# TimoLassmann/kalign

Measured on AMD Instinct MI355X. Metric: GCUPS (DP cell updates/s) on NxL synthetic MSA, higher is better.
Workload: dtype f32

## Files before the change

kalign_amd/csrc/ka_api.cpp:

```cpp
#include "ka_ctx.h"
#include "ka_marks.h"

static thread_local std::string g_err;
int fail(const std::string& m) { g_err = m; return KA_FAIL; }
__attribute__((visibility("hidden"))) int ka_fail_message(const char* m) { return fail(m); }

extern "C" const char* ka_last_error(void) { return g_err.c_str(); }
struct ka_ctx;
int ka_ctx_device_stream(ka_ctx* c, int* device, hipStream_t* stream);
extern "C" int ka_abi_version(void) { return 29; }

extern "C" int ka_ctx_create(int device, ka_ctx** out)
{
        int n = 0;
        if (hipGetDeviceCount(&n) != hipSuccess || n <= 0) return fail("no HIP device visible (the HIP path has no CPU fallback)");
        if (device < 0 || device >= n) return fail("bad device index");
        HIPCHK(hipSetDevice(device));
        ka_ctx* c = new ka_ctx();
        c->device = device;
        {
                hipDeviceProp_t prop;
                if (hipGetDeviceProperties(&prop, device) == hipSuccess && prop.multiProcessorCount > 0) c->n_cus = prop.multiProcessorCount;
        }
        hipError_t e = hipEventCreate(&c->ev0);
// ... 159 lines not shown
        D.scratch = c->d_scratch.p; D.path_arena = c->d_path_arena.p;
        D.dbg_arena = c->d_dbg_arena.p; D.dbg_off = c->d_dbg_off.p;
        D.tasks = c->d_tasks.p; D.recs = c->d_recs.p; D.subm = c->d_subm.p;
        D.ctl = (KaCtl*)c->d_ctl.p;
        D.join = c->d_join.p;
        D.gpo0 = c->scal[0]; D.gpe0 = c->scal[1]; D.tgpe0 = c->scal[2]; D.usw = c->scal[5];
        D.numseq = c->numseq; D.flags = c->flags; D.error = c->d_error.p;
        D.nres = c->nres;
        D.trace = c->h_trace;
        D.refine_mode = 0;
        D.refine_adaptive = 0;
        D.refine_trials = 3;
        D.prof_task = -1;
        D.wdfs = (c->env.no_wdfs ? 0 : 1) | (c->env.no_ls0 ? 0 : 2) | (c->env.no_inc ? 0 : 4) | (c->env.no_ldfs ? 0 : 8);
        D.prof_task = c->env.prof_task;
        D.timing = (c->flags & KA_FLAG_TIMING) ? c->d_timing.p : nullptr;
        D.max_g = std::max(1, std::min(c->max_cluster, ka_max_g_host()));
        D.q1_mode = c->env.q1 >= 0 ? c->env.q1 : (c->nres > 5 ? 4 : 0);
        D.ho_mode = c->env.ho >= 0 ? c->env.ho : 1;
        D.per_target = c->env.per;
        D.q_order = nullptr; D.q_n = 0; D.q_slots = 0; D.qw = c->env.qw; D.lw = c->env.lw; D.reuse = c->env.reuse;
        D.overlap = c->overlap_plan ? 1 : 0;
        D.hw_mode = c->env.hw ? (1 | (c->env.hw_prio << 4)) : 0;
        D.lean4 = c->env.lean4;
        D.sub_mode = c->env.subtree;
        D.mw_mode = c->env.mw;
        D.merge_batch = c->env.merge;
        D.cons_K = c->cons_K; D.cons_maxlen = c->max_len;
        D.cons_paw = c->cons_K > 0 ? c->cons_weight / (float)c->cons_K : 0.0f;
        D.cons_maps = c->d_cons_maps.p; D.cons_map_off = c->d_cons_map_off.p;
        D.colof = c->d_colof.p; D.sip = c->d_sip.p; D.sip_off = c->d_sip_off.p;
        return D;
}

static int mark_launch(ka_ctx* c, hipStream_t s = nullptr)
{
        if (!c->env.launch_ev) return KA_OK;
        while ((int)c->launch_ev.size() < c->n_launches) { hipEvent_t e; HIPCHK(hipEventCreate(&e)); c->launch_ev.push_back(e); }
        HIPCHK(hipEventRecord(c->launch_ev[c->n_launches - 1], s ? s : c->stream));
        return KA_OK;
}

static int launch_chain(ka_ctx* c, const KaTreeDev& D, bool ov, bool join_now = true)
{
        hipStream_t cs = ov ? c->s_chain : c->stream;
        KaTreeDev Dc = D;
// ... 1165 lines not shown
```

kalign_amd/csrc/ka_device.h:

```cpp
#pragma once
#include <stdint.h>
#include "kalign_amd.h"

#define KA_F 3.402823466e+38f
#define KA_REC 64

enum { KA_SS = 0, KA_SP = 1, KA_PP = 2 };
enum { KA_FWD = 0, KA_BWD = 1 };

struct KaState { float a, ga, gb; };

struct KaTaskDesc {
        int a, b, c;
        int nsip_a, nsip_b;
        int is_root;
        float gpo, gpe, tgpe;
        float soff;
        float gap_scale;
        int parent;
        int chain_need;
        int qa, qb;
        int wait_mult;
        int refine;
};
// ... 49 lines not shown
        int* error;
        int max_g;
        int mw_mode;
        int sub_mode;
        int lean4;
        int q1_mode;
        int ho_mode;
        int hw_mode;
        int reuse;
        int overlap;
        const int2* q_order;
        int q_n, q_slots;
        int qw, lw;
        int per_target;
        int cons_K;
        int cons_maxlen;
        float cons_paw;
        const int* cons_maps;
        const long long* cons_map_off;
        int* colof;
        const int* sip;
        const long long* sip_off;
        int merge_batch;
};

#define KA_NB 6
#define KA_NB_BIG 136

struct KaPairDev {
        const uint8_t* codes;
        const int* seq_off;
        const int* seq_len;
        const int* ia;
        const int* ib;
        const float* subm;
        float gpo, gpe, tgpe;
        char* scratch;
        long long scratch_stride;
        int* paths_out;
        const long long* poff;
        float* scores;
        int* error;
        int npairs;
        int pw;
        int reuse;
};
// ... 1 lines not shown
```

kalign_amd/csrc/ka_hirschberg.h:

```cpp
#pragma once

__device__ void ka_cluster_sync(TaskShared& S)
{
        __syncthreads();
        if (S.G == 1 || S.split) return;
        if (threadIdx.x == 0) {
                __builtin_amdgcn_fence(__ATOMIC_RELEASE, "agent");
                asm volatile("s_waitcnt vmcnt(0)" ::: "memory");
                S.bar_phase += 1;
                const unsigned int target = S.bar_phase * (unsigned int)S.G;
                __hip_atomic_fetch_add(&S.ctl->bar, 1u, __ATOMIC_RELAXED, __HIP_MEMORY_SCOPE_AGENT);
                int spins = 0;
                while (__hip_atomic_load(&S.ctl->bar, __ATOMIC_RELAXED, __HIP_MEMORY_SCOPE_AGENT) < target) {
                        __builtin_amdgcn_s_sleep(4);
                        if (ka_spin_expired(S.watchdog, ++spins, 1 << 24, 6)) break;
                }
                __builtin_amdgcn_fence(__ATOMIC_ACQUIRE, "agent");
        }
        __syncthreads();
}

#define KA_CRUMB(D_trace, slot, val) do { if (D_trace) { ((volatile int*)(D_trace))[slot] = (val); __threadfence_system(); } } while (0)


template <int KIND, int NRES, int NB, bool Q1 = false, bool HO = false, bool HW = false, bool RU = false>
__device__ __forceinline__ void ka_run_items(TaskShared& S, KaCtl::Lvl* const cur, const int level, const KaSub* qc, char* lds_waves,
                                             const float* tss, long long* pslot)
{
        const int tid = threadIdx.x;
        const int lane = tid & 63;
        const int wave = tid >> 6;
        {
                        const int2* items = S.items[level & 1];
                        int* prog = S.prog[level & 1];
                        const int nitems = cur->nitems;
                        const int n16 = cur->npack[0], n4 = cur->npack[1];
                        const int njobs16 = (n16 + 3) / 4, njobs4 = (n4 + 15) / 16;
                        const int2* pack16 = S.pack[level & 1][0];
                        const int2* pack4 = S.pack[level & 1][1];
                        const int ntotal = nitems + njobs16 + njobs4;
                        const int Gw = __builtin_amdgcn_readfirstlane(S.Gw), member_w = __builtin_amdgcn_readfirstlane(S.member_w);
                        const int nslots = __builtin_amdgcn_readfirstlane(KA_NW * Gw);
                        int nreg = 1;
                        if (ntotal <= nslots) {
                                const int per_wg = (ntotal + Gw - 1) / Gw;
// ... 720 lines not shown
```

kalign_amd/csrc/ka_pass.h:

```cpp
#pragma once

#include <type_traits>

typedef float float2v __attribute__((ext_vector_type(2)));
typedef float float4v __attribute__((ext_vector_type(4)));

#define KA_STRIP_ROWS 128
#define KA_STRIP1_ROWS 64
#define KA_RING_BATCH 32
#define KA_RING_SLOTS 4
#define KA_REC_CHUNKS 7
#define KA_SLOT_BYTES (KA_REC_CHUNKS * KA_RING_BATCH * 16)
#define KA_RING_BYTES (KA_RING_SLOTS * KA_SLOT_BYTES)
#define KA_WAVE_LDS 18432
#define KA_SP_STRIDE 25
#define KA_PK_RECS 128
#define KA_SP_FILL 23
#define KA_WAVE_LDS_LEAN 6144
#define KA_T_STRIDE 24

#ifndef KA_BONUS_ASM
#define KA_BONUS_ASM 1
#endif
#ifndef KA_UNTRACKED_READS
#define KA_UNTRACKED_READS 0
#endif
#define KA_WAIT_VM0 0x0F70

typedef __attribute__((address_space(3))) void* ka_lds_ptr;
typedef const __attribute__((address_space(1))) void* ka_glb_ptr;
typedef __attribute__((address_space(1))) float ka_gfloat;
typedef const __attribute__((address_space(1))) float4v ka_gfloat4c;
typedef const __attribute__((address_space(1))) unsigned char ka_gbytec;

__device__ __forceinline__ int wave_shr1_i(int x)
{
        return __builtin_amdgcn_update_dpp(x, x, 0x138, 0xf, 0xf, false);
}

__device__ __forceinline__ float wave_shr1_old(float old, float src)
{
        return __int_as_float(__builtin_amdgcn_update_dpp(__float_as_int(old), __float_as_int(src), 0x138, 0xf, 0xf, false));
}
__device__ __forceinline__ float wave_shl1_old(float old, float src)
{
        return __int_as_float(__builtin_amdgcn_update_dpp(__float_as_int(old), __float_as_int(src), 0x130, 0xf, 0xf, false));
}
template <int E>
__device__ __forceinline__ float2v ka_mul_bcast(const float2v a, const float4v& v)
{
// ... 171 lines not shown

        const unsigned wlds_u = (unsigned)(unsigned long long)wlds;
        auto ring_issue = [&](int nb) {
                if (lane < KA_RING_BATCH && nb * KA_RING_BATCH <= ncols) {
                        const int vv = min(nb * KA_RING_BATCH + lane, ncols);
                        const float* g = p2u + ((long long)REC(vv) << 6) + 32;
                        char* dst = wlds + (nb & (KA_RING_SLOTS - 1)) * (KA_RING_BATCH * 16);
#pragma unroll
                        for (int ch = 0; ch < KA_REC_CHUNKS; ++ch)
                                if (ka_chunk_used<NRES>(ch))
                                        __builtin_amdgcn_global_load_lds((ka_glb_ptr)(g + 4 * ch), (ka_lds_ptr)(dst + ch * 2048), 16, 0, 0);
                }
        };
        if (KIND == KA_PP) {
                __builtin_amdgcn_s_waitcnt(KA_WAIT_VM0);
                ring_issue(0);
                ring_issue(1);
        }
        float oA, eA, tA, oB, eB, tB, orpA, orpB;
        float2v p1v[Q == 2 ? NRES : 1];
        constexpr int NPAIR = NRES / 2;
        float2v p1p[Q == 1 ? (NPAIR > 0 ? NPAIR : 1) : 1];
        float p1last = 0.0f;
        int res1A = 0, res1B = 0;
        if (KIND == KA_SS) {
                oA = oB = -S.gpo; eA = eB = -S.gpe; tA = tB = -S.tgpe; orpA = orpB = -S.gpo;
                res1A = S.s1[iA] * KA_T_STRIDE; res1B = S.s1[iB] * KA_T_STRIDE;
        } else {
                const float* pA = S.p1 + ((long long)recA << 6);
                const float* pB = S.p1 + ((long long)recB << 6);
                oA = pA[55] * m1; eA = pA[56] * m1; tA = pA[57] * m1;
                oB = pB[55] * m1; eB = pB[56] * m1; tB = pB[57] * m1;
                orpA = S.p1[((long long)prevA << 6) + 55] * m1;
                orpB = S.p1[((long long)prevB << 6) + 55] * m1;
                if (KIND == KA_PP) {
                        constexpr int NV = (NRES + 3) / 4;
                        if constexpr (Q == 2) {
                                float4v va[NV], vb[NV];
#pragma unroll
                                for (int i = 0; i < NV; ++i) { va[i] = ((const float4v*)pA)[i]; vb[i] = ((const float4v*)pB)[i]; }
#pragma unroll
                                for (int c = 0; c < NRES; ++c) {
                                        p1v[c].x = va[c >> 2][c & 3];
                                        p1v[c].y = actB ? vb[c >> 2][c & 3] : 0.0f;
                                }
                        } else {
                                float4v va[NV];
#pragma unroll
                                for (int i = 0; i < NV; ++i) va[i] = ((const float4v*)pA)[i];
#pragma unroll
                                for (int i = 0; i < NPAIR; ++i) { p1p[i].x = va[(2 * i) >> 2][(2 * i) & 3]; p1p[i].y = va[(2 * i + 1) >> 2][(2 * i + 1) & 3]; }
                                if (NRES & 1) p1last = va[(NRES - 1) >> 2][(NRES - 1) & 3];
                        }
                } else {
                        float* tA_ = sp_tbl + (Q * lane) * KA_SP_STRIDE;
                        float4v sa[6];
#pragma unroll
                        for (int i = 0; i < 6; ++i) sa[i] = ((const float4v*)(pA + 32))[i];
#pragma unroll
                        for (int c = 0; c < KA_SP_FILL; ++c) tA_[c] = sa[c >> 2][c & 3];
                        if constexpr (Q == 2) {
                                float* tB_ = tA_ + KA_SP_STRIDE;
                                float4v sb[6];
#pragma unroll
                                for (int i = 0; i < 6; ++i) sb[i] = ((const float4v*)(pB + 32))[i];
#pragma unroll
                                for (int c = 0; c < KA_SP_FILL; ++c) tB_[c] = sb[c >> 2][c & 3];
// ... 49 lines not shown
                             "ds_read_b128 %5, %8 offset:10240\n\t"
                             "ds_read_b128 %6, %8 offset:12288"
                             : "=&v"(dstq[0]), "=&v"(dstq[1]), "=&v"(dstq[2]), "=&v"(dstq[3]), "=&v"(dstq[4]), "=&v"(dstq[5]), "=&v"(dstq[6]),
                               "+v"(dep)
                             : "v"(a)
                             : "memory");
        };
        auto ring_wait = [&](float4v* qq) {
                if (!KA_UNTRACKED_READS) {
                        if (NRES <= 8) asm volatile("" : "+v"(qq[0]), "+v"(qq[1]), "+v"(qq[5]), "+v"(qq[6]) : : "memory");
                        else asm volatile("" : "+v"(qq[0]), "+v"(qq[1]), "+v"(qq[2]), "+v"(qq[3]), "+v"(qq[4]), "+v"(qq[5]), "+v"(qq[6]) : : "memory");
                        return;
                }
                if (NRES <= 8) {
                        asm volatile("s_waitcnt lgkmcnt(0)" : "+v"(qq[0]), "+v"(qq[1]), "+v"(qq[5]), "+v"(qq[6]) : : "memory");
                        return;
                }
                asm volatile("s_waitcnt lgkmcnt(0)"
                             : "+v"(qq[0]), "+v"(qq[1]), "+v"(qq[2]), "+v"(qq[3]), "+v"(qq[4]), "+v"(qq[5]), "+v"(qq[6])
                             :
                             : "memory");
        };

        const unsigned ho_out_u = wlds_u + KA_HO_RING;
        const unsigned ho_in_u = wlds_u - KA_WAVE_LDS + KA_HO_RING;
        const unsigned ho_my_u = (unsigned)(unsigned long long)ho_ctl_w;
        auto lds_word = [&](const unsigned addr) -> int {
                int x;
                asm volatile("ds_read_b32 %0, %1\n\ts_waitcnt lgkmcnt(0)" : "=&v"(x) : "v"(addr) : "memory");
                return __builtin_amdgcn_readfirstlane(x);
        };
        auto lds_wait_for = [&](const unsigned addr, const int need) {
                int spins = 0;
                while (lds_word(addr) < need) {
                        __builtin_amdgcn_s_sleep(1);
                        if (ka_spin_expired(wdu, ++spins, 1 << 22, 5)) break;
                }
        };

        if (KIND == KA_PP) {
                __builtin_amdgcn_s_waitcnt(KA_WAIT_VM0);
                { float2v nodep = {0.0f, 0.0f}; ring_read(q[0], min(max(-lane, 0), ncols), nodep); }
        } else {
                resn = ((ka_gbytec*)s2u)[REC(min(1 + lane, ncols)) - 1];
                if (KIND == KA_SS) { scA = tss[res1A]; if (Q == 2) scB = tss[res1B]; }
                else { scA = sp_tbl[(Q * lane) * KA_SP_STRIDE]; if (Q == 2) scB = sp_tbl[(2 * lane + 1) * KA_SP_STRIDE]; }
        }

#ifdef KA_PROF
        if (pslot && lane == 0 && pslot[2] == 0) pslot[2] = __builtin_amdgcn_s_memtime();
#endif
        auto step = [&](const int t, auto st_tag, auto full_tag, auto par_tag, auto ev_tag, auto first_tag, auto lb_tag) {
                constexpr bool LASTB = decltype(lb_tag)::value;
                constexpr bool FIRST = decltype(first_tag)::value;
                constexpr bool ST = decltype(st_tag)::value;
                constexpr bool FULL = decltype(full_tag)::value;
                constexpr int P = decltype(par_tag)::value;
                constexpr bool EV = decltype(ev_tag)::value;
                const int v = t - lane;
#ifdef KA_PROF
                const long long tq0 = __builtin_amdgcn_s_memtime();
#endif

                float copen, cext, ctext;
                if (KIND == KA_PP) {
                        ring_wait(q[P]);
#ifdef KA_PROF
                        if (EV && ST && pslot && lane == 0) pslot[256 + 0] += __builtin_amdgcn_s_memtime() - tq0;
#endif
                        copen = q[P][5].w * m2; cext = q[P][6].x * m2; ctext = q[P][6].y * m2;
                } else {
                        copen = kc_open; cext = kc_ext; ctext = kc_text;
                }
                const float scA_cur = scA, scB_cur = scB;
                if (KIND != KA_PP) {
                        if (EV && (t & 63) == 0) {
                                resb = resn;
                                resn = ((ka_gbytec*)s2u)[REC(min(t + 65 + lane, ncols)) - 1];
                        } else {
                                resb = __builtin_amdgcn_update_dpp(resb, resb, 0x134, 0xf, 0xf, false);
                        }
                        res2 = __builtin_amdgcn_update_dpp(resb, res2, 0x138, 0xf, 0xf, false);
                        if (KIND == KA_SS) { scA = tss[res1A + res2]; if (Q == 2) scB = tss[res1B + res2]; }
                        else { scA = sp_tbl[(Q * lane) * KA_SP_STRIDE + res2]; if (Q == 2) scB = sp_tbl[(2 * lane + 1) * KA_SP_STRIDE + res2]; }
                }

                if (FIRST) {
                        if (!ST && t == 0) {
                                inia = inj_a; iniga = inj_ga; inigb = inj_gb;
// ... 44 lines not shown
                }
                float upa, upga, upgb;
                const float lra = (Q == 2) ? cBa : cAa, lrga = (Q == 2) ? cBga : cAga, lrgb = (Q == 2) ? cBgb : cAgb;
                if (FIRST) {
                        upa = wave_shr1_old(bta, lra); upga = wave_shr1_old(btga, lrga); upgb = wave_shr1_old(btgb, lrgb);
                } else {
                        const float nbta = wave_rol1(bta), nbtga = wave_rol1(btga), nbtgb = wave_rol1(btgb);
                        upa = wave_shr1_old(bta, lra); upga = wave_shr1_old(btga, lrga); upgb = wave_shr1_old(btgb, lrgb);
                        bta = nbta; btga = nbtga; btgb = nbtgb;
                }

                if constexpr (Q == 2) {
                        float2v acc;
                        acc.x = kmax3(dga, dgga + copen_prev, dggb + orpA);
                        acc.y = kmax3(cAa, cAga + copen_prev, cAgb + orpB);
                        if (KIND == KA_SS) {
                                acc.x += scA_cur;
                                acc.y += scB_cur;
                                if (NB) { const int jb = (dir == KA_FWD) ? (startb + v) : (endb - v); acc.x += bonA.template at<!ST>(jb); acc.y += bonB.template at<!ST>(jb); }
                        } else if (KIND == KA_SP) {
                                acc.x += scA_cur;
                                acc.y += scB_cur;
                                if (NB) { const int jb = (dir == KA_FWD) ? (startb + v) : (endb - v); acc.x += bonA.template at<!ST>(jb); acc.y += bonB.template at<!ST>(jb); }
                        } else {
                                float2v prod;
                                prod = ka_mul_bcast<(NRES - 1) & 3>(p1v[NRES - 1], q[P][(NRES - 1) >> 2]);
        #pragma unroll
                                for (int c = NRES - 1; c >= 1; --c) {
                                        float2v nprod;
                                        switch ((c - 1) & 3) {
                                        case 0: nprod = ka_mul_bcast<0>(p1v[c - 1], q[P][(c - 1) >> 2]); break;
                                        case 1: nprod = ka_mul_bcast<1>(p1v[c - 1], q[P][(c - 1) >> 2]); break;
                                        case 2: nprod = ka_mul_bcast<2>(p1v[c - 1], q[P][(c - 1) >> 2]); break;
                                        default: nprod = ka_mul_bcast<3>(p1v[c - 1], q[P][(c - 1) >> 2]); break;
                                        }
                                        acc = acc + prod;
                                        prod = nprod;
                                }
                                acc = acc + prod;
                                if (NB) { const int jb = (dir == KA_FWD) ? (startb + v) : (endb - v); acc.x += bonA.template at<!ST>(jb); acc.y += bonB.template at<!ST>(jb); }
                                {
                                __builtin_amdgcn_sched_barrier(0);
                                const int tn = t + 1;
#ifdef KA_PROF
                                const long long tq2 = __builtin_amdgcn_s_memtime();
#endif
// ... 124 lines not shown
                                } else if (rel_agent) {
                                        __builtin_amdgcn_fence(__ATOMIC_RELEASE, "agent");
                                        asm volatile("s_waitcnt vmcnt(0)" ::: "memory");
                                        if (lane == 0) __hip_atomic_store(prog + k, vL + 1, __ATOMIC_RELAXED, __HIP_MEMORY_SCOPE_AGENT);
                                } else {
                                        __builtin_amdgcn_fence(__ATOMIC_RELEASE, "workgroup");
                                        if (lane == 0) __hip_atomic_store(prog + k, vL + 1, __ATOMIC_RELAXED, __HIP_MEMORY_SCOPE_WORKGROUP);
                                }
                                }
                        }
                }
#ifdef KA_PROF
                if (EV && ST && pslot && lane == 0) pslot[256 + 7] += __builtin_amdgcn_s_memtime() - tfl0_outer;
#endif
#ifdef KA_PROF
                const long long tri0 = __builtin_amdgcn_s_memtime();
#endif
                if (KIND == KA_PP && EV && ((t + 1) & (KA_RING_BATCH - 1)) == 0) ring_issue(((t + 1) >> 5) + 1);
#ifdef KA_PROF
                if (EV && ST && pslot && lane == 0) pslot[256 + 6] += __builtin_amdgcn_s_memtime() - tri0;
#endif
        };

        auto run = [&](int& t, const int tend, auto st_tag, auto full_tag, auto first_tag, auto lb_tag) {
                constexpr bool FIRST = decltype(first_tag)::value;
                const int e4 = ncols + lastl;
                while (t < tend) {
                        const int e1 = t | 31;
                        const int e2 = (KIND == KA_PP && FIRST) ? 0x7fffffff : ((t + CBM) & ~CBM);
                        const int e3 = t + ((lastl - t) & PBM);
                        const int e5 = (t <= e4) ? e4 : 0x7fffffff;
                        const int ev = min(min(e1, e2), min(e3, e5));
                        const int fend = min(ev, tend);
                        if ((t & 1) && t < fend) {
                                step(t, st_tag, full_tag, std::integral_constant<int, 1>(), std::false_type(), first_tag, lb_tag);
                                ++t;
                        }
                        for (; t + 1 < fend; t += 2) {
                                step(t, st_tag, full_tag, std::integral_constant<int, 0>(), std::false_type(), first_tag, lb_tag);
                                step(t + 1, st_tag, full_tag, std::integral_constant<int, 1>(), std::false_type(), first_tag, lb_tag);
                        }
                        if (t < fend) {
                                step(t, st_tag, full_tag, std::integral_constant<int, 0>(), std::false_type(), first_tag, lb_tag);
                                ++t;
                        }
                        if (t < tend && t == ev) {
                                if (t & 1) step(t, st_tag, full_tag, std::integral_constant<int, 1>(), std::true_type(), first_tag, lb_tag);
                                else step(t, st_tag, full_tag, std::integral_constant<int, 0>(), std::true_type(), first_tag, lb_tag);
                                ++t;
                        }
                }
        };
        auto run_steady = [&](int& t, const int tend, auto full_tag, auto first_tag, auto lb_tag) {
                constexpr bool FIRST = decltype(first_tag)::value;
                while (t < tend) {
                        const int e1 = t | 31;
                        const int e2 = (KIND == KA_PP && FIRST) ? 0x7fffffff : ((t + CBM) & ~CBM);
                        const int e3 = t + ((lastl - t) & PBM);
                        const int ev = min(e1, min(e2, e3));
                        const int fend = min(ev, tend);
                        if ((t & 1) && t < fend) {
                                step(t, std::true_type(), full_tag, std::integral_constant<int, 1>(), std::false_type(), first_tag, lb_tag);
                                ++t;
                        }
#ifdef KA_PROF
                        const long long tpair0 = __builtin_amdgcn_s_memtime();
                        const int t_in = t;
#endif
                        for (; t + 1 < fend; t += 2) {
                                step(t, std::true_type(), full_tag, std::integral_constant<int, 0>(), std::false_type(), first_tag, lb_tag);
                                step(t + 1, std::true_type(), full_tag, std::integral_constant<int, 1>(), std::false_type(), first_tag, lb_tag);
                        }
#ifdef KA_PROF
                        if (pslot && lane == 0) { pslot[6] += __builtin_amdgcn_s_memtime() - tpair0; pslot[7] += t - t_in; }
#endif
                        if (t < fend) {
                                step(t, std::true_type(), full_tag, std::integral_constant<int, 0>(), std::false_type(), first_tag, lb_tag);
                                ++t;
                        }
#ifdef KA_PROF
                        const long long tev0 = __builtin_amdgcn_s_memtime();
                        const int ev_in = t;
#endif
                        if (t < tend && t == ev) {
                                if (t & 1) step(t, std::true_type(), full_tag, std::integral_constant<int, 1>(), std::true_type(), first_tag, lb_tag);
                                else step(t, std::true_type(), full_tag, std::integral_constant<int, 0>(), std::true_type(), first_tag, lb_tag);
                                ++t;
                        }
#ifdef KA_PROF
                        if (pslot && lane == 0) { pslot[256 + 2] += __builtin_amdgcn_s_memtime() - tev0; pslot[256 + 3] += t - ev_in; }
#endif
                }
        };

        const int nsteps = ncols + nl;
        const int t_steady0 = min(nl, nsteps);
        const int t_steady1 = ncols;
        auto phases = [&](auto full_tag, auto first_tag, auto lb_tag) {
                int t = 0;
                run(t, t_steady0, std::false_type(), full_tag, first_tag, lb_tag);
                run_steady(t, t_steady1, full_tag, first_tag, lb_tag);
                run(t, nsteps, std::false_type(), full_tag, first_tag, lb_tag);
        };
        auto go = [&](auto full_tag, auto first_tag) {
                constexpr bool FULL = decltype(full_tag)::value;
                if constexpr (FULL || Q == 1) phases(full_tag, first_tag, std::integral_constant<bool, Q == 2>());
                else { if (last_is_b) phases(full_tag, first_tag, std::true_type()); else phases(full_tag, first_tag, std::false_type()); }
        };
        if (nr == SROWS) {
                if (first) go(std::true_type(), std::true_type());
                else go(std::true_type(), std::false_type());
        } else {
                if (first) go(std::false_type(), std::true_type());
                else go(std::false_type(), std::false_type());
        }
#undef REC
#undef IDX
}

template <int KIND, int NRES, int SLOT, int NB>
__device__ __forceinline__ void ka_packed(const TaskShared& S, const KaSub* qc, const int2* pack, const int nslots,
                                          const int job, const int lane, const float* tss, char* wlds,
                                          const int nreg = 1, const int reg_stride = 0)
{
        constexpr int SPW = 64 / SLOT;
        const int slot = job * SPW + lane / SLOT;
        const int ls = lane % SLOT;
        const bool live = slot < nslots;
        const int2 d = pack[live ? slot : 0];
        const KaSub* sp = qc + d.x;
        const int dir = d.y;
        const int starta = sp->starta, enda = sp->enda, startb = sp->startb, endb = sp->endb;
        const int ncols = endb - startb;
        const int mid = ((enda - starta) / 2) + starta;
        const int r0 = (dir == KA_FWD) ? starta : mid;
        const int r1 = (dir == KA_FWD) ? mid : enda;
        const int nrows = r1 - r0;
// ... 202 lines not shown
```

kalign_amd/csrc/ka_plan.h:

```cpp
#pragma once
#define KA_INTERNAL __attribute__((visibility("hidden")))

#include <algorithm>
#include <cstdlib>
#include <string>
#include <vector>

#include "ka_device.h"

KA_INTERNAL int fail(const std::string& m);

struct KaEnv {
        bool trace = false, no_chain = false, no_queue = false, no_half = false, no_lean = false, chain_g1 = false, no_crit = false;
        bool no_staging = false, no_wdfs = false, no_ls0 = false, no_inc = false, no_ldfs = false, refine_serial = false;
        int chain_tasks = 0;
        int max_cluster = 0;
        int crit_greedy = 1;
        int crit_top = 0;
        int prof_task = -1;
        int q1 = -1;
        int lean4 = 1;
        int mw = 1;
        int merge = 15;
        int per = 0;
        int ho = -1;
        int hw = 1;
        int hw_prio = 3;
        int subtree = 1;
        int overlap = 1;
        int overlap_help = 1;
        int reuse = 1;
        int qw = 4, lw = 4, pw = 2;
        bool launch_ev = false;
        bool upgma_launches = false;
        bool qorder = true;
        bool plan_verbose = false;
};
static inline int env_int(const char* name, int dflt) { const char* e = getenv(name); return e ? atoi(e) : dflt; }
static inline void read_env(KaEnv& v)
{
        v = KaEnv();
        v.trace = getenv("KA_TRACE") != nullptr; v.no_chain = getenv("KA_NO_CHAIN") != nullptr; v.no_queue = getenv("KA_NO_QUEUE") != nullptr;
        v.no_half = getenv("KA_NO_HALF") != nullptr; v.no_lean = getenv("KA_NO_LEAN") != nullptr; v.chain_g1 = getenv("KA_CHAIN_G1") != nullptr;
        v.no_crit = getenv("KA_NO_CRIT") != nullptr; v.no_staging = getenv("KA_NO_STAGING") != nullptr;
        v.no_wdfs = getenv("KA_NO_WDFS") != nullptr; v.no_ls0 = getenv("KA_NO_LS0") != nullptr; v.no_inc = getenv("KA_NO_INC") != nullptr; v.no_ldfs = getenv("KA_NO_LDFS") != nullptr; v.refine_serial = getenv("KA_REFINE_SERIAL") != nullptr;
        v.chain_tasks = env_int("KA_CHAIN_TASKS", 0); v.max_cluster = env_int("KA_MAX_CLUSTER", 0); v.crit_top = env_int("KA_CRIT_TOP", 0); v.crit_greedy = env_int("KA_CRIT_GREEDY", 1);
        v.prof_task = env_int("KA_PROF_TASK", -1); v.q1 = env_int("KA_Q1", -1); v.lean4 = env_int("KA_LEAN4", 1);
        v.launch_ev = getenv("KA_LAUNCH_EV") != nullptr;
        v.subtree = env_int("KA_SUBTREE", 1);
        v.reuse = env_int("KA_REUSE", 1);
        v.overlap_help = env_int("KA_OVERLAP_HELP", 1);
        v.overlap = env_int("KA_OVERLAP", 1);
        v.qw = env_int("KA_QW", 4); v.lw = env_int("KA_LW", 4); v.pw = env_int("KA_PW", 2);
        for (int* w : { &v.qw, &v.lw, &v.pw }) if (*w != 1 && *w != 2) *w = 4;
        v.mw = env_int("KA_MW", 1);
        v.merge = env_int("KA_MERGE", 15);
        v.ho = env_int("KA_HO", -1);
        v.per = env_int("KA_PER", 0);
        v.hw = env_int("KA_HW", 1);
        v.hw_prio = std::max(0, std::min(3, env_int("KA_HW_PRIO", 3)));
        v.upgma_launches = getenv("KA_UPGMA_LAUNCHES") != nullptr;
        v.qorder = env_int("KA_QORDER", 1) != 0;
        v.plan_verbose = getenv("KA_PLAN_VERBOSE") != nullptr;
}

struct KaPlan {
        KaEnv env;
        int numseq = 0, n_tasks = 0;
        std::vector<int> lens;
        std::vector<int> abc;
        std::vector<KaTaskDesc> descs;
        std::vector<std::vector<int>> levels;
        std::vector<int> task_level;
        std::vector<int> sip_flat;
        std::vector<long long> sip_off;
        std::vector<char> plan_active;
        int n_cus = 256;
        bool shared_gpu = false;
        int cons_K = 0;
        int test_hooks = 0;
        std::vector<std::vector<int>> plan_levels;
        std::vector<int2> blocks_flat;
// ... 16 lines not shown
```

kalign_amd/csrc/ka_shared.h:

```cpp
#pragma once

#define KA_BLOCK 512
#define KA_WAVES (KA_BLOCK / 64)
#define KA_PAIR_BLOCK 256
#define KA_LEAN_BLOCK 512
#define KA_NT ((int)blockDim.x)
#define KA_NW ((int)blockDim.x >> 6)

__device__ __forceinline__ float kmax(float a, float b) { return fmaxf(a, b); }
__device__ __forceinline__ float kmax3(float a, float b, float c) { return fmaxf(fmaxf(a, b), c); }

__device__ __forceinline__ float wave_shr1(float x)
{
        int xi = __float_as_int(x);
        return __int_as_float(__builtin_amdgcn_update_dpp(xi, xi, 0x138, 0xf, 0xf, false));
}

__device__ __forceinline__ float ka_uniform_f(float x)
{
        return __int_as_float(__builtin_amdgcn_readfirstlane(__float_as_int(x)));
}

template <typename T>
__device__ __forceinline__ T* ka_uniform_ptr(T* p)
// ... 11 lines not shown
        return false;
}

__device__ __forceinline__ float lane_bcast(float x, int src_lane)
{
        return __int_as_float(__builtin_amdgcn_readlane(__float_as_int(x), src_lane));
}

struct KaCtl {
        struct Lvl { int nsub, rowalloc, nitems, next_item, npack[2], next_job, pad; } lvl[2];
        int mcount;
        int top_meet, top_tr;
        float top_score;
        double msum;
        int alnlen;
        int fail;
        unsigned int bar;
        int nrec;
        long long scratch_off;
        long long newp_off;
        long long path_off;
        int regalloc_pad[2];
};

struct TaskShared {
        int kind, swapped;
        int len_a, len_b;
        int La, Lb;
        const uint8_t* s1;
        const uint8_t* s2;
        const float* p1;
        const float* p2;
        float* profa;
        float* profb;
        const float* subm;
        float gpo, gpe, tgpe, soff;
        float sp_open, sp_ext, sp_text;
        float p1_mult, p2_mult;
        KaState* fbuf;
        KaState* bbuf;
        KaState* xfbuf;
        KaState* xbbuf;
        KaState* sfbuf[2];
        KaState* sbbuf[2];
        int reuse_ok;
        KaSub* q[2];
// ... 32 lines not shown
        float* mlog;
        int mlog_cap, adapt_trials;
        int2* mrec;
        char* inc;
        int inc_n, inc_nunc;
        int inc_j, inc_p;
        int rec_on;
        float sp_value;
        int Gw, member_w;
        int split;
        struct Priv { KaSub* q[2]; int2* items[2]; int* prog[2]; int2* pack[2][2]; KaState* f; KaState* b; } priv;
        unsigned int bar_phase;
        int2* items[2];
        int* prog[2];
        int2* pack[2][2];
        float* newp;
        int* path_dst;
        int* trace;
        int dbgskip;
        int* watchdog;
        long long t_pass, t_meet;
        int n_levels;
        int next_member, next_g;
        long long* prof;
        int lvl_n[16];
        int lvl_pass[16], lvl_meet[16];
};

template <int KIND>
__device__ __forceinline__ void col_terms(const TaskShared& S, int rec, float& copen, float& cext, float& ctext)
{
        if (KIND == KA_SS) { copen = -S.gpo; cext = -S.gpe; ctext = -S.tgpe; }
        else if (KIND == KA_SP) { copen = -S.sp_open; cext = -S.sp_ext; ctext = -S.sp_text; }
        else {
                const float* c = S.p2 + ((long long)rec << 6);
                copen = c[55] * S.p2_mult; cext = c[56] * S.p2_mult; ctext = c[57] * S.p2_mult;
        }
}
```

kalign_amd/csrc/ka_task.h:

```cpp
#pragma once

#ifndef KA_RU_TREE
#define KA_RU_TREE 0
#endif
#define KA_LDS_DBG 1400
#define KA_LDS_TSS 1408
#define KA_LDS_WAVES 4096
static_assert(KA_LDS_TSS + 23 * KA_T_STRIDE * 4 <= KA_LDS_WAVES - KA_LDS_HO_BACK, "score table overlaps the hand-over control words");
static_assert(KA_LDS_TSS + 23 * KA_T_STRIDE * 4 <= KA_LDS_WAVES, "score table overlaps the wave regions");
#define KA_LDS_TOTAL (KA_LDS_WAVES + KA_WAVES * KA_WAVE_LDS)
#define KA_HALF_BLOCK 256
#define KA_LDS_HALF (KA_LDS_WAVES + (KA_HALF_BLOCK / 64) * KA_WAVE_LDS)
#define KA_LEAN_SCRATCH(nt_) ((((2 * (nt_) + 16) * 4) + 15) & ~15)
#define KA_LDS_PAIR (KA_LDS_WAVES + KA_LEAN_SCRATCH(KA_PAIR_BLOCK) + (KA_PAIR_BLOCK / 64) * KA_WAVE_LDS_LEAN)
#define KA_LDS_LEAN (KA_LDS_WAVES + KA_LEAN_SCRATCH(KA_LEAN_BLOCK) + (KA_LEAN_BLOCK / 64) * KA_WAVE_LDS_LEAN)
static_assert(sizeof(TaskShared) <= KA_LDS_DBG, "TaskShared outgrew its LDS slot");
static_assert(KA_LDS_WAVES % 16 == 0, "wave regions must be 16-B aligned");

__device__ void ka_build_tss(float* tss, const float* subm, float soff)
{
        for (int x = threadIdx.x; x < 23 * KA_T_STRIDE; x += KA_NT) {
                const int a = x / KA_T_STRIDE, b = x % KA_T_STRIDE;
                tss[x] = (b < 23) ? (subm[23 * a + b] - soff) : 0.0f;
        }
// ... 194 lines not shown
                S.kind = kind; S.swapped = swapped;
                S.p1_mult = swapped ? (float)T.nsip_a : (float)T.nsip_b;
                S.p2_mult = swapped ? (float)T.nsip_b : (float)T.nsip_a;
                S.La = swapped ? len_b : len_a;
                S.Lb = swapped ? len_a : len_b;
                int g_eff = (S.La >= 1536) ? 8 : ((S.La >= 1152) ? 6 : ((S.La >= 768) ? 4 : ((S.La >= 320) ? 2 : 1)));
                int srows = KA_STRIP_ROWS;
                int q1_lvl = 0;
                if (Q1 && D.q1_mode == 4) {
                        if (D.hw_mode && kind == KA_PP) {
                                const int s1 = ka_strips_of(S.La / 2, KA_STRIP1_ROWS) + ka_strips_of(S.La - S.La / 2, KA_STRIP1_ROWS);
                                q1_lvl = 1;
                                g_eff = max(g_eff, min(g_launch, (s1 + 3) / 4));
                        }
                } else if (Q1 && D.q1_mode) {
                        const int s1 = ka_strips_of(S.La / 2, KA_STRIP1_ROWS) + ka_strips_of(S.La - S.La / 2, KA_STRIP1_ROWS);
                        const int g1 = (s1 + 3) / 4;
                        if (g1 <= g_launch || (D.q1_mode >= 2 && (s1 + 7) / 8 <= g_launch) || D.q1_mode >= 3) { srows = KA_STRIP1_ROWS; g_eff = g1; }
                }
                S.q1_lvl = q1_lvl;
                S.lvl_srows[0] = srows; S.lvl_srows[1] = srows;
                S.ho_ok = (Q1 && NB == 0 && D.ho_mode && kind == KA_PP) ? 1 : 0;
                S.hw_ok = (Q1 && D.hw_mode && kind == KA_PP) ? D.hw_mode : 0;
                if (Q1 && kind == KA_PP) {
                        const int s2 = ka_strips_of(S.La / 2, srows) + ka_strips_of(S.La - S.La / 2, srows);
                        g_eff = (S.ho_ok && D.ho_mode >= 2) ? max((s2 + 3) / 4, 1) : max(g_eff, (s2 + 3) / 4);
                        if (S.hw_ok && !q1_lvl) {
                                int need = s2;
                                for (int l = 1; l < 5; ++l) {
                                        const int rows = (S.La + (2 << l) - 1) >> (l + 1);
                                        if (rows < 2 * srows) break;
                                        need = max(need, (2 << l) * ka_strips_of(rows, srows));
                                }
                                g_eff = max(g_eff, min(g_launch, (need + 3) / 4));
                        }
                }
                if (Q1 && D.per_target > 0 && kind == KA_PP) {
                        const int s2 = ka_strips_of(S.La / 2, srows) + ka_strips_of(S.La - S.La / 2, srows);
                        g_eff = max((s2 + D.per_target - 1) / D.per_target, 1);
                }
                if (NB && D.cons_K > 0 && T.nsip_a + T.nsip_b >= 128) {
                        const int mem = max(T.nsip_a, T.nsip_b);
                        g_eff = max(g_eff, 2 * D.cons_K * (mem >= 1536 ? 3 : (mem >= 384 ? 2 : 1)));
                }
                if (g_eff > g_launch) g_eff = g_launch;
                S.srows = srows;
// ... 515 lines not shown
```

Baseline: 56.03.

## Add gathered sparse profile scoring path for low-residue-count PP rows

Adds a specialised profile-profile DP step that, when every lane's row profile has at most four nonzero residue columns, gathers only those columns from the LDS ring and computes the match score with a few multiply-adds instead of the dense NRES-wide dot product. The choice is made per strip through a wave-wide ballot, and the whole pass loop is instantiated twice via a template tag. This targets per-cell ALU and LDS read cost on near-identical synthetic MSAs, at the cost of larger code, extra register pressure, and a path that only runs in the KA_UNIT==2 build.

```diff
diff --git a/kalign_amd/csrc/ka_api.cpp b/kalign_amd/csrc/ka_api.cpp
--- a/kalign_amd/csrc/ka_api.cpp
+++ b/kalign_amd/csrc/ka_api.cpp
@@ -205,6 +205,7 @@
         D.q_order = nullptr; D.q_n = 0; D.q_slots = 0; D.qw = c->env.qw; D.lw = c->env.lw; D.reuse = c->env.reuse;
         D.overlap = c->overlap_plan ? 1 : 0;
         D.hw_mode = c->env.hw ? (1 | (c->env.hw_prio << 4)) : 0;
+        D.sparse_mode = c->env.sparse ? 1 : 0;
         D.lean4 = c->env.lean4;
         D.sub_mode = c->env.subtree;
         D.mw_mode = c->env.mw;
diff --git a/kalign_amd/csrc/ka_device.h b/kalign_amd/csrc/ka_device.h
--- a/kalign_amd/csrc/ka_device.h
+++ b/kalign_amd/csrc/ka_device.h
@@ -95,6 +95,7 @@
         const int* sip;
         const long long* sip_off;
         int merge_batch;
+        int sparse_mode;
 };
 
 #define KA_NB 6
diff --git a/kalign_amd/csrc/ka_hirschberg.h b/kalign_amd/csrc/ka_hirschberg.h
--- a/kalign_amd/csrc/ka_hirschberg.h
+++ b/kalign_amd/csrc/ka_hirschberg.h
@@ -20,7 +20,6 @@
         __syncthreads();
 }
 
-#define KA_CRUMB(D_trace, slot, val) do { if (D_trace) { ((volatile int*)(D_trace))[slot] = (val); __threadfence_system(); } } while (0)
 
 
 template <int KIND, int NRES, int NB, bool Q1 = false, bool HO = false, bool HW = false, bool RU = false>
diff --git a/kalign_amd/csrc/ka_pass.h b/kalign_amd/csrc/ka_pass.h
--- a/kalign_amd/csrc/ka_pass.h
+++ b/kalign_amd/csrc/ka_pass.h
@@ -26,6 +26,15 @@
 #define KA_UNTRACKED_READS 0
 #endif
 #define KA_WAIT_VM0 0x0F70
+
+#ifndef KA_SPARSE_NT
+#define KA_SPARSE_NT 4
+#endif
+#if defined(KA_UNIT) && KA_UNIT == 2
+#define KA_SPARSE_BUILT 1
+#else
+#define KA_SPARSE_BUILT 0
+#endif
 
 typedef __attribute__((address_space(3))) void* ka_lds_ptr;
 typedef const __attribute__((address_space(1))) void* ka_glb_ptr;
@@ -243,6 +252,12 @@
         constexpr int NPAIR = NRES / 2;
         float2v p1p[Q == 1 ? (NPAIR > 0 ? NPAIR : 1) : 1];
         float p1last = 0.0f;
+        constexpr bool SPB = KA_SPARSE_BUILT && KIND == KA_PP && NRES >= 20 && NB == 0 && Q == 2;
+        constexpr int SP_NTMAX = SPB ? KA_SPARSE_NT : 1;
+        static_assert(!SPB || !KA_UNTRACKED_READS, "the gathered form reads the ring with tracked loads only");
+        int sp_nt = 0;
+        float2v spc[SP_NTMAX];
+        unsigned spo[SP_NTMAX];
         int res1A = 0, res1B = 0;
         if (KIND == KA_SS) {
                 oA = oB = -S.gpo; eA = eB = -S.gpe; tA = tB = -S.tgpe; orpA = orpB = -S.gpo;
@@ -260,10 +275,33 @@
                                 float4v va[NV], vb[NV];
 #pragma unroll
                                 for (int i = 0; i < NV; ++i) { va[i] = ((const float4v*)pA)[i]; vb[i] = ((const float4v*)pB)[i]; }
-#pragma unroll
-                                for (int c = 0; c < NRES; ++c) {
-                                        p1v[c].x = va[c >> 2][c & 3];
-                                        p1v[c].y = actB ? vb[c >> 2][c & 3] : 0.0f;
+                                if constexpr (SPB) {
+                                        unsigned nz = 0;
+#pragma unroll
+                                        for (int c = 0; c < NRES; ++c)
+                                                if (va[c >> 2][c & 3] != 0.0f || (actB && vb[c >> 2][c & 3] != 0.0f)) nz |= 1u << c;
+                                        const int nterms = __popc(nz);
+                                        if (__builtin_amdgcn_readfirstlane(S.sparse_ok) != 0 && __ballot(nterms > KA_SPARSE_NT) == 0ull) sp_nt = KA_SPARSE_NT;
+                                        if (S.trace && lane == 0) ((volatile int*)S.trace)[sp_nt ? KA_TRACE_GATHERED : KA_TRACE_DENSE] = 1;
+                                        if (sp_nt) {
+#pragma unroll
+                                                for (int i = 0; i < SP_NTMAX; ++i) {
+                                                        const bool has = nz != 0u;
+                                                        const int c = has ? 31 - __clz(nz) : 0;
+                                                        nz &= ~(1u << c);
+                                                        const float xa = pA[c], xb = pB[c];
+                                                        spc[i].x = has ? xa : 0.0f;
+                                                        spc[i].y = (has && actB) ? xb : 0.0f;
+                                                        spo[i] = wlds_u + (unsigned)((c >> 2) * 2048 + (c & 3) * 4);
+                                                }
+                                        }
+                                }
+                                if (!SPB || sp_nt == 0) {
+#pragma unroll
+                                        for (int c = 0; c < NRES; ++c) {
+                                                p1v[c].x = va[c >> 2][c & 3];
+                                                p1v[c].y = actB ? vb[c >> 2][c & 3] : 0.0f;
+                                        }
                                 }
                         } else {
                                 float4v va[NV];
@@ -359,6 +397,25 @@
                              : "memory");
         };
 
+        float sq[2][SP_NTMAX];
+        auto sp_read = [&](float4v* dstq, float* dsts, int vcol, auto& dep, auto n_tag) {
+                constexpr int N = decltype(n_tag)::value;
+                typedef const __attribute__((address_space(3))) float4v ka_l4;
+                typedef const __attribute__((address_space(3))) float ka_l1;
+                const unsigned cb = ((unsigned)vcol & 127u) << 4;
+                ka_l4* const cr = (ka_l4*)(unsigned long)(wlds_u | cb);
+                asm volatile("" : "+v"(dep) : : "memory");
+#pragma unroll
+                for (int i = 0; i < N; ++i) dsts[i] = *(ka_l1*)(unsigned long)(spo[i] | cb);
+                dstq[5] = cr[5 * 128]; dstq[6] = cr[6 * 128];
+        };
+        auto sp_wait = [&](float4v* qq, float* ss, auto n_tag) {
+                constexpr int N = decltype(n_tag)::value;
+#pragma unroll
+                for (int i = 0; i < N; ++i) asm volatile("" : "+v"(ss[i]) : : "memory");
+                asm volatile("" : "+v"(qq[5]), "+v"(qq[6]) : : "memory");
+        };
+
         const unsigned ho_out_u = wlds_u + KA_HO_RING;
         const unsigned ho_in_u = wlds_u - KA_WAVE_LDS + KA_HO_RING;
         const unsigned ho_my_u = (unsigned)(unsigned long long)ho_ctl_w;
@@ -377,7 +434,11 @@
 
         if (KIND == KA_PP) {
                 __builtin_amdgcn_s_waitcnt(KA_WAIT_VM0);
-                { float2v nodep = {0.0f, 0.0f}; ring_read(q[0], min(max(-lane, 0), ncols), nodep); }
+                float2v nodep = {0.0f, 0.0f};
+                bool gathered = false;
+                if constexpr (SPB) gathered = sp_nt != 0;
+                if (gathered) sp_read(q[0], sq[0], min(max(-lane, 0), ncols), nodep, std::integral_constant<int, SP_NTMAX>());
+                else ring_read(q[0], min(max(-lane, 0), ncols), nodep);
         } else {
                 resn = ((ka_gbytec*)s2u)[REC(min(1 + lane, ncols)) - 1];
                 if (KIND == KA_SS) { scA = tss[res1A]; if (Q == 2) scB = tss[res1B]; }
@@ -387,7 +448,8 @@
 #ifdef KA_PROF
         if (pslot && lane == 0 && pslot[2] == 0) pslot[2] = __builtin_amdgcn_s_memtime();
 #endif
-        auto step = [&](const int t, auto st_tag, auto full_tag, auto par_tag, auto ev_tag, auto first_tag, auto lb_tag) {
+        auto step = [&](const int t, auto st_tag, auto full_tag, auto par_tag, auto ev_tag, auto first_tag, auto lb_tag, auto nt_tag) {
+                constexpr int NTV = decltype(nt_tag)::value;
                 constexpr bool LASTB = decltype(lb_tag)::value;
                 constexpr bool FIRST = decltype(first_tag)::value;
                 constexpr bool ST = decltype(st_tag)::value;
@@ -401,7 +463,7 @@
 
                 float copen, cext, ctext;
                 if (KIND == KA_PP) {
-                        ring_wait(q[P]);
+                        if constexpr (NTV > 0) sp_wait(q[P], sq[P], nt_tag); else ring_wait(q[P]);
 #ifdef KA_PROF
                         if (EV && ST && pslot && lane == 0) pslot[256 + 0] += __builtin_amdgcn_s_memtime() - tq0;
 #endif
@@ -492,6 +554,21 @@
                                 acc.x += scA_cur;
                                 acc.y += scB_cur;
                                 if (NB) { const int jb = (dir == KA_FWD) ? (startb + v) : (endb - v); acc.x += bonA.template at<!ST>(jb); acc.y += bonB.template at<!ST>(jb); }
+                        } else if constexpr (NTV > 0) {
+                                float2v prod;
+                                { float2v w; w.x = sq[P][0]; w.y = sq[P][0]; prod = spc[0] * w; }
+#pragma unroll
+                                for (int i = 1; i < NTV; ++i) {
+                                        float2v w; w.x = sq[P][i]; w.y = sq[P][i];
+                                        const float2v nprod = spc[i] * w;
+                                        acc = acc + prod;
+                                        prod = nprod;
+                                }
+                                acc = acc + prod;
+                                __builtin_amdgcn_sched_barrier(0);
+                                if (EV && ((t + 1) & (KA_RING_BATCH - 1)) == 0) __builtin_amdgcn_s_waitcnt(KA_WAIT_VM0);
+                                sp_read(q[1 - P], sq[1 - P], ST ? (v + 1) : min(max(v + 1, 0), ncols), acc, nt_tag);
+                                __builtin_amdgcn_sched_barrier(0);
                         } else {
                                 float2v prod;
                                 prod = ka_mul_bcast<(NRES - 1) & 3>(p1v[NRES - 1], q[P][(NRES - 1) >> 2]);
@@ -662,7 +739,7 @@
 #endif
         };
 
-        auto run = [&](int& t, const int tend, auto st_tag, auto full_tag, auto first_tag, auto lb_tag) {
+        auto run = [&](int& t, const int tend, auto st_tag, auto full_tag, auto first_tag, auto lb_tag, auto nt_tag) {
                 constexpr bool FIRST = decltype(first_tag)::value;
                 const int e4 = ncols + lastl;
                 while (t < tend) {
@@ -673,25 +750,25 @@
                         const int ev = min(min(e1, e2), min(e3, e5));
                         const int fend = min(ev, tend);
                         if ((t & 1) && t < fend) {
-                                step(t, st_tag, full_tag, std::integral_constant<int, 1>(), std::false_type(), first_tag, lb_tag);
+                                step(t, st_tag, full_tag, std::integral_constant<int, 1>(), std::false_type(), first_tag, lb_tag, nt_tag);
                                 ++t;
                         }
                         for (; t + 1 < fend; t += 2) {
-                                step(t, st_tag, full_tag, std::integral_constant<int, 0>(), std::false_type(), first_tag, lb_tag);
-                                step(t + 1, st_tag, full_tag, std::integral_constant<int, 1>(), std::false_type(), first_tag, lb_tag);
+                                step(t, st_tag, full_tag, std::integral_constant<int, 0>(), std::false_type(), first_tag, lb_tag, nt_tag);
+                                step(t + 1, st_tag, full_tag, std::integral_constant<int, 1>(), std::false_type(), first_tag, lb_tag, nt_tag);
                         }
                         if (t < fend) {
-                                step(t, st_tag, full_tag, std::integral_constant<int, 0>(), std::false_type(), first_tag, lb_tag);
+                                step(t, st_tag, full_tag, std::integral_constant<int, 0>(), std::false_type(), first_tag, lb_tag, nt_tag);
                                 ++t;
                         }
                         if (t < tend && t == ev) {
-                                if (t & 1) step(t, st_tag, full_tag, std::integral_constant<int, 1>(), std::true_type(), first_tag, lb_tag);
-                                else step(t, st_tag, full_tag, std::integral_constant<int, 0>(), std::true_type(), first_tag, lb_tag);
+                                if (t & 1) step(t, st_tag, full_tag, std::integral_constant<int, 1>(), std::true_type(), first_tag, lb_tag, nt_tag);
+                                else step(t, st_tag, full_tag, std::integral_constant<int, 0>(), std::true_type(), first_tag, lb_tag, nt_tag);
                                 ++t;
                         }
                 }
         };
-        auto run_steady = [&](int& t, const int tend, auto full_tag, auto first_tag, auto lb_tag) {
+        auto run_steady = [&](int& t, const int tend, auto full_tag, auto first_tag, auto lb_tag, auto nt_tag) {
                 constexpr bool FIRST = decltype(first_tag)::value;
                 while (t < tend) {
                         const int e1 = t | 31;
@@ -700,7 +777,7 @@
                         const int ev = min(e1, min(e2, e3));
                         const int fend = min(ev, tend);
                         if ((t & 1) && t < fend) {
-                                step(t, std::true_type(), full_tag, std::integral_constant<int, 1>(), std::false_type(), first_tag, lb_tag);
+                                step(t, std::true_type(), full_tag, std::integral_constant<int, 1>(), std::false_type(), first_tag, lb_tag, nt_tag);
                                 ++t;
                         }
 #ifdef KA_PROF
@@ -708,14 +785,14 @@
                         const int t_in = t;
 #endif
                         for (; t + 1 < fend; t += 2) {
-                                step(t, std::true_type(), full_tag, std::integral_constant<int, 0>(), std::false_type(), first_tag, lb_tag);
-                                step(t + 1, std::true_type(), full_tag, std::integral_constant<int, 1>(), std::false_type(), first_tag, lb_tag);
+                                step(t, std::true_type(), full_tag, std::integral_constant<int, 0>(), std::false_type(), first_tag, lb_tag, nt_tag);
+                                step(t + 1, std::true_type(), full_tag, std::integral_constant<int, 1>(), std::false_type(), first_tag, lb_tag, nt_tag);
                         }
 #ifdef KA_PROF
                         if (pslot && lane == 0) { pslot[6] += __builtin_amdgcn_s_memtime() - tpair0; pslot[7] += t - t_in; }
 #endif
                         if (t < fend) {
-                                step(t, std::true_type(), full_tag, std::integral_constant<int, 0>(), std::false_type(), first_tag, lb_tag);
+                                step(t, std::true_type(), full_tag, std::integral_constant<int, 0>(), std::false_type(), first_tag, lb_tag, nt_tag);
                                 ++t;
                         }
 #ifdef KA_PROF
@@ -723,8 +800,8 @@
                         const int ev_in = t;
 #endif
                         if (t < tend && t == ev) {
-                                if (t & 1) step(t, std::true_type(), full_tag, std::integral_constant<int, 1>(), std::true_type(), first_tag, lb_tag);
-                                else step(t, std::true_type(), full_tag, std::integral_constant<int, 0>(), std::true_type(), first_tag, lb_tag);
+                                if (t & 1) step(t, std::true_type(), full_tag, std::integral_constant<int, 1>(), std::true_type(), first_tag, lb_tag, nt_tag);
+                                else step(t, std::true_type(), full_tag, std::integral_constant<int, 0>(), std::true_type(), first_tag, lb_tag, nt_tag);
                                 ++t;
                         }
 #ifdef KA_PROF
@@ -736,23 +813,31 @@
         const int nsteps = ncols + nl;
         const int t_steady0 = min(nl, nsteps);
         const int t_steady1 = ncols;
-        auto phases = [&](auto full_tag, auto first_tag, auto lb_tag) {
+        auto phases = [&](auto full_tag, auto first_tag, auto lb_tag, auto nt_tag) {
                 int t = 0;
-                run(t, t_steady0, std::false_type(), full_tag, first_tag, lb_tag);
-                run_steady(t, t_steady1, full_tag, first_tag, lb_tag);
-                run(t, nsteps, std::false_type(), full_tag, first_tag, lb_tag);
-        };
-        auto go = [&](auto full_tag, auto first_tag) {
+                run(t, t_steady0, std::false_type(), full_tag, first_tag, lb_tag, nt_tag);
+                run_steady(t, t_steady1, full_tag, first_tag, lb_tag, nt_tag);
+                run(t, nsteps, std::false_type(), full_tag, first_tag, lb_tag, nt_tag);
+        };
+        auto go = [&](auto full_tag, auto first_tag, auto nt_tag) {
                 constexpr bool FULL = decltype(full_tag)::value;
-                if constexpr (FULL || Q == 1) phases(full_tag, first_tag, std::integral_constant<bool, Q == 2>());
-                else { if (last_is_b) phases(full_tag, first_tag, std::true_type()); else phases(full_tag, first_tag, std::false_type()); }
-        };
-        if (nr == SROWS) {
-                if (first) go(std::true_type(), std::true_type());
-                else go(std::true_type(), std::false_type());
+                if constexpr (FULL || Q == 1) phases(full_tag, first_tag, std::integral_constant<bool, Q == 2>(), nt_tag);
+                else { if (last_is_b) phases(full_tag, first_tag, std::true_type(), nt_tag); else phases(full_tag, first_tag, std::false_type(), nt_tag); }
+        };
+        auto go_form = [&](auto nt_tag) __attribute__((always_inline)) {
+                if (nr == SROWS) {
+                        if (first) go(std::true_type(), std::true_type(), nt_tag);
+                        else go(std::true_type(), std::false_type(), nt_tag);
+                } else {
+                        if (first) go(std::false_type(), std::true_type(), nt_tag);
+                        else go(std::false_type(), std::false_type(), nt_tag);
+                }
+        };
+        if constexpr (SPB) {
+                if (sp_nt != 0) go_form(std::integral_constant<int, KA_SPARSE_NT>());
+                else go_form(std::integral_constant<int, 0>());
         } else {
-                if (first) go(std::false_type(), std::true_type());
-                else go(std::false_type(), std::false_type());
+                go_form(std::integral_constant<int, 0>());
         }
 #undef REC
 #undef IDX
diff --git a/kalign_amd/csrc/ka_plan.h b/kalign_amd/csrc/ka_plan.h
--- a/kalign_amd/csrc/ka_plan.h
+++ b/kalign_amd/csrc/ka_plan.h
@@ -25,6 +25,7 @@
         int per = 0;
         int ho = -1;
         int hw = 1;
+        int sparse = 1;
         int hw_prio = 3;
         int subtree = 1;
         int overlap = 1;
@@ -58,6 +59,7 @@
         v.ho = env_int("KA_HO", -1);
         v.per = env_int("KA_PER", 0);
         v.hw = env_int("KA_HW", 1);
+        v.sparse = env_int("KA_SPARSE", 1);
         v.hw_prio = std::max(0, std::min(3, env_int("KA_HW_PRIO", 3)));
         v.upgma_launches = getenv("KA_UPGMA_LAUNCHES") != nullptr;
         v.qorder = env_int("KA_QORDER", 1) != 0;
diff --git a/kalign_amd/csrc/ka_shared.h b/kalign_amd/csrc/ka_shared.h
--- a/kalign_amd/csrc/ka_shared.h
+++ b/kalign_amd/csrc/ka_shared.h
@@ -57,6 +57,10 @@
         long long path_off;
         int regalloc_pad[2];
 };
+
+#define KA_CRUMB(D_trace, slot, val) do { if (D_trace) { ((volatile int*)(D_trace))[slot] = (val); __threadfence_system(); } } while (0)
+#define KA_TRACE_GATHERED 60
+#define KA_TRACE_DENSE 61
 
 struct TaskShared {
         int kind, swapped;
@@ -135,10 +139,12 @@
         long long t_pass, t_meet;
         int n_levels;
         int next_member, next_g;
+        int sparse_ok;
         long long* prof;
         int lvl_n[16];
         int lvl_pass[16], lvl_meet[16];
 };
+static_assert(offsetof(TaskShared, sparse_ok) + 4 == offsetof(TaskShared, prof) && offsetof(TaskShared, sparse_ok) == offsetof(TaskShared, next_g) + 4, "sparse_ok left the padding it was put into");
 
 template <int KIND>
 __device__ __forceinline__ void col_terms(const TaskShared& S, int rec, float& copen, float& cext, float& ctext)
diff --git a/kalign_amd/csrc/ka_task.h b/kalign_amd/csrc/ka_task.h
--- a/kalign_amd/csrc/ka_task.h
+++ b/kalign_amd/csrc/ka_task.h
@@ -240,6 +240,9 @@
                 S.lvl_srows[0] = srows; S.lvl_srows[1] = srows;
                 S.ho_ok = (Q1 && NB == 0 && D.ho_mode && kind == KA_PP) ? 1 : 0;
                 S.hw_ok = (Q1 && D.hw_mode && kind == KA_PP) ? D.hw_mode : 0;
+#if KA_SPARSE_BUILT
+                if constexpr (NB == 0) S.sparse_ok = D.sparse_mode;
+#endif
                 if (Q1 && kind == KA_PP) {
                         const int s2 = ka_strips_of(S.La / 2, srows) + ka_strips_of(S.La - S.La / 2, srows);
                         g_eff = (S.ho_ok && D.ho_mode >= 2) ? max((s2 + 3) / 4, 1) : max(g_eff, (s2 + 3) / 4);
```

After: 56.84 (median of 6 runs). 1.01x the previous value.
